# MarvelMathesh/sincformer-metacog-speech-enhancement

Measured on AMD Instinct MI355X. Metric: audio frames/sec/GPU (16 kHz, 512-frame utts) + mask RMSE vs CPU ref, higher is better.
Workload: dtype fp16 MFMA operands (PerceptionAgent, fusion, Conformer GEMMs, heads) + bf16 attention core, fp32 accumulate (ops.POLICIES['mixed']); 1 GPU; B256 x 512-frame utterances (L40880, T512) forward; batch_per_gpu=256, samples=40880, frames_per_utt=512, launch=eager launches, streams=3, precision_policy=mixed

## Files before the change

### sincformer_metacog_speech_enhancement_amd/csrc/headpool.hip

```cpp
#include "sfm_common.h"

#define HP_BM 128
#define HP_K 256
#define HP_STAGE 32768
#define HP_NSTAGE 3
#define HP_IMG 16384


template <class T>
__global__ __launch_bounds__(512) void headpool_kernel(const u16* __restrict__ A, const u16* __restrict__ W,
                                                       const float* __restrict__ bias, u16* __restrict__ pooled,
                                                       float* __restrict__ gn_partial, int Tin, int Tout, int NW, int lda,
                                                       int ldp, int fpt, int P, int gcols, int w_bytes, int p_bytes) {
  extern __shared__ __attribute__((aligned(16))) unsigned char smem[];
  unsigned char* img0 = smem + HP_NSTAGE * HP_STAGE;
  float* bs = reinterpret_cast<float*>(img0 + 2 * HP_IMG);
  float* st = bs + NW;

  const int tid = threadIdx.x, lane = tid & 63;
  const int wave = __builtin_amdgcn_readfirstlane(tid >> 6);
  const int l31 = lane & 31, hl = lane >> 5;
  const int j = blockIdx.x % P, b = blockIdx.x / P;
  const int i0 = j * fpt, i1 = min(i0 + fpt, Tout);
  const int r_lo = (int)(((long long)i0 * Tin) / Tout);
  const int own_end = (j + 1 < P) ? (int)(((long long)i1 * Tin) / Tout) : Tin;
  const int nch = NW >> 6;
  const int ngr = NW / gcols;
  auto a_rs = __builtin_amdgcn_make_buffer_rsrc((void*)(A + (long long)b * Tin * lda), 0, Tin * lda * 2, 0x00020000);
  auto w_rs = __builtin_amdgcn_make_buffer_rsrc((void*)W, 0, w_bytes, 0x00020000);
  auto p_rs = __builtin_amdgcn_make_buffer_rsrc((void*)pooled, 0, p_bytes, 0x00020000);

#pragma unroll
  for (int i = 0; i < 8; ++i) {
    const int inst = wave * 8 + i;
    const int row = inst * 2 + (lane >> 5);
    const int lc = (lane & 31) ^ (row & 15);
    const int r = r_lo + row;
    __builtin_amdgcn_raw_ptr_buffer_load_lds(a_rs, (lds_ptr_t)(smem + inst * 1024), 16,
                                             r < Tin ? (r * lda + lc * 8) * 2 : Tin * lda * 2, 0, 0, 0);
  }
  for (int i = tid; i < NW; i += 512) bs[i] = bias ? bias[i] : 0.f;
  wait_vmcnt<0>();
  __syncthreads();
  const int r1 = (wave >> 1) * 32 + l31;
  u32x4 hf[16];
#pragma unroll
  for (int s = 0; s < 16; ++s) hf[s] = *reinterpret_cast<const u32x4*>(smem + r1 * 512 + (((2 * s + hl) ^ (r1 & 15)) << 4));
  __syncthreads();

  auto w_piece = [&](int c, int stage, int i) {
    const int inst = wave * 4 + i;
    const int row = inst * 2 + (lane >> 5);
    const int lc = (lane & 31) ^ (row & 15);
    const int voff = c < nch ? ((c * 64 + row) * HP_K + lc * 8) * 2 : w_bytes;
    __builtin_amdgcn_raw_ptr_buffer_load_lds(w_rs, (lds_ptr_t)(smem + stage * HP_STAGE + inst * 1024), 16, voff, 0, 0, 0);
  };
#pragma unroll
  for (int c = 0; c < 3; ++c)
#pragma unroll
    for (int i = 0; i < 4; ++i) w_piece(c, c, i);

  const int half = wave & 1;
  const int n1 = half * 32 + l31;
  const uint32_t w_lane = (uint32_t)(uintptr_t)(lds_ptr_t)smem + (uint32_t)(n1 * 512);
  const int hx4 = (hl ^ (n1 & 15)) << 4;
  const bool own = (r_lo + r1) < own_end;
  float gs[2] = {0.f, 0.f}, gq[2] = {0.f, 0.f};
  auto epi_quad = [&](const f32x16& s, int c, int q) {
    const f32x4 bv = *reinterpret_cast<const f32x4*>(bs + c * 64 + half * 32 + 8 * q + 4 * hl);
    float y[4];
#pragma unroll
    for (int e = 0; e < 4; ++e) y[e] = s[4 * q + e] + bv[e];
    u32x2 pk;
    pk[0] = pack2<T>(y[0], y[1]);
    pk[1] = pack2<T>(y[2], y[3]);
    const int col = half * 32 + 8 * q + 4 * hl;
    unsigned char* img = img0 + ((c & 1) ? HP_IMG : 0);
    *reinterpret_cast<u32x2*>(img + r1 * 128 + (((col >> 3) ^ ((r1 >> 1) & 7)) << 4) + (col & 7) * 2) = pk;
    if (own) {
      const int g = (8 * q) / gcols;
#pragma unroll
      for (int e = 0; e < 4; ++e) {
        gs[g] += y[e];
        gq[g] = __builtin_fmaf(y[e], y[e], gq[g]);
      }
    }
  };
  auto stats_out = [&](int c) {
#pragma unroll
    for (int g = 0; g < 2; ++g) {
      const float a = wave_sum_dpp(gs[g]), q2 = wave_sum_dpp(gq[g]);
      if (lane == 0) {
        float* d = st + (((wave >> 1) * ngr + (c * 64 + half * 32) / gcols + g) << 1);
        d[0] = a;
        d[1] = q2;
      }
      gs[g] = 0.f;
      gq[g] = 0.f;
    }
  };
  const int pf = tid >> 4, pc = tid & 15;
  const int fi = i0 + pf;
  int ws = 0, we = 0;
  if (fi < i1) {
    ws = (int)(((long long)fi * Tin) / Tout) - r_lo;
    we = (int)((((long long)(fi + 1)) * Tin + Tout - 1) / Tout) - r_lo;
  }
  const float winv = we > ws ? 1.0f / (float)(we - ws) : 0.f;
  auto pool_chunk = [&](int c) {
    const unsigned char* img = img0 + ((c & 1) ? HP_IMG : 0);
    float a[4] = {0.f, 0.f, 0.f, 0.f};
    for (int r = ws; r < we; ++r) {
      const u32x2 v = *reinterpret_cast<const u32x2*>(img + r * 128 + (((pc >> 1) ^ ((r >> 1) & 7)) << 4) + (pc & 1) * 8);
#pragma unroll
      for (int e = 0; e < 2; ++e) {
        const uint32_t w = v[e];
        a[2 * e] += T::to_f32((u16)(w & 0xffffu));
        a[2 * e + 1] += T::to_f32((u16)(w >> 16));
      }
    }
    u32x2 pk;
    pk[0] = pack2<T>(a[0] * winv, a[1] * winv);
    pk[1] = pack2<T>(a[2] * winv, a[3] * winv);
    const int voff = (fi < i1) ? (((b * Tout + fi) * ldp) + c * 64 + pc * 4) * 2 : p_bytes;
    __builtin_amdgcn_raw_buffer_store_b64(pk, p_rs, voff, 0, 0);
  };

  wait_vmcnt<8>();
  ring_barrier();
  f32x16 s1;
#pragma unroll
  for (int r = 0; r < 16; ++r) s1[r] = 0.f;
  {
    u32x4 fw[4];
#pragma unroll
    for (int k = 0; k < 4; ++k) fw[k] = *reinterpret_cast<const u32x4*>(smem + n1 * 512 + (((2 * k + hl) ^ (n1 & 15)) << 4));
#pragma unroll
    for (int k = 0; k < 16; ++k) {
      s1 = T::mfma(fw[k & 3], hf[k], s1);
      if (k + 4 < 16) fw[k & 3] = *reinterpret_cast<const u32x4*>(smem + n1 * 512 + (((2 * (k + 4) + hl) ^ (n1 & 15)) << 4));
    }
  }
  wait_vmcnt<4>();
  ring_barrier();

  int stage_next = 1, stage_free = 0;
  for (int c = 0; c + 1 < nch; ++c) {
    if (c >= 1) pool_chunk(c - 1);
    f32x16 s1n;
#pragma unroll
    for (int r = 0; r < 16; ++r) s1n[r] = 0.f;
    const uint32_t fbase = w_lane + (uint32_t)(stage_next * HP_STAGE);
    u32x4 fw[4];
#pragma unroll
    for (int k = 0; k < 4; ++k) frag_read(fw[k], fbase + (uint32_t)(hx4 ^ (k << 5)));
#pragma unroll
    for (int k = 0; k < 16; ++k) {
      if (k <= 12) frag_wait<3>(fw[k & 3]);
      else if (k == 13) frag_wait<2>(fw[k & 3]);
      else if (k == 14) frag_wait<1>(fw[k & 3]);
      else frag_wait<0>(fw[k & 3]);
      s1n = T::mfma(fw[k & 3], hf[k], s1n);
      if (k + 4 < 16) frag_read(fw[k & 3], fbase + (uint32_t)(hx4 ^ ((k + 4) << 5)));
      if ((k & 3) == 1) epi_quad(s1, c, k >> 2);
      if ((k & 3) == 3) w_piece(c + 3, stage_free, k >> 2);
    }
    stats_out(c);
    s1 = s1n;
    if (c >= 1) wait_vmcnt<5>();
    else wait_vmcnt<4>();
    ring_barrier();
    stage_free = stage_next;
    stage_next = (stage_next == HP_NSTAGE - 1) ? 0 : stage_next + 1;
  }
  if (nch >= 2) pool_chunk(nch - 2);
#pragma unroll
  for (int q = 0; q < 4; ++q) epi_quad(s1, nch - 1, q);
  stats_out(nch - 1);
  wait_vmcnt<0>();
  ring_barrier();
  pool_chunk(nch - 1);
  if (tid < ngr * 2) {
    const float v = ((st[tid] + st[ngr * 2 + tid]) + st[2 * ngr * 2 + tid]) + st[3 * ngr * 2 + tid];
    gn_partial[((long long)b * P + j) * ngr * 2 + tid] = v;
  }
}

extern "C" int sfm_headpool_frames_per_tile(int Tin, int Tout) {
  if (Tin <= 0 || Tout <= 0 || Tin < Tout) return 0;
  for (int f = 32; f >= 1; --f) {
    bool ok = true;
    for (int i0 = 0; i0 < Tout && ok; i0 += f) {
      const int i1 = i0 + f < Tout ? i0 + f : Tout;
      const long long lo = ((long long)i0 * Tin) / Tout, hi = (((long long)i1) * Tin + Tout - 1) / Tout;
      if (hi - lo > HP_BM) ok = false;
    }
    if (ok) return f;
  }
  return 0;
}

extern "C" int sfm_headpool(const void* xd, const void* W, const float* bias, void* pooled, float* gn_partial, int B, int Tin,
                            int Tout, int NW, int lda, int ldp, int gcols, int dtype, void* stream) {
  if (!xd || !W || !pooled || !gn_partial) return SFM_ERR_ARG;
  if (dtype != SFM_DT_BF16 && dtype != SFM_DT_F16) return SFM_ERR_ARG;
  const int fpt = sfm_headpool_frames_per_tile(Tin, Tout);
  if (B <= 0 || fpt <= 0 || NW <= 0 || (NW % 64) != 0 || NW > 1024 || gcols != 16 || lda < HP_K || (lda % 8) != 0 || (ldp % 4) != 0 ||
      ldp < NW)
    return SFM_ERR_SHAPE;
  const int P = (Tout + fpt - 1) / fpt;
  const long long p_bytes = (long long)B * Tout * ldp * 2, a_b = (long long)Tin * lda * 2;
  if (p_bytes >= (1LL << 31) || a_b >= (1LL << 31) || (long long)B * P > 2147483647LL) return SFM_ERR_SHAPE;
  const int ngr = NW / gcols;
  const int lds = HP_NSTAGE * HP_STAGE + 2 * HP_IMG + NW * 4 + 4 * ngr * 2 * 4;
  const int w_bytes = NW * HP_K * 2;
  dim3 grid(B * P), block(512);
  hipStream_t st = (hipStream_t)stream;
#define HP_GO(TT) SFM_LAUNCH_LDS((headpool_kernel<TT>), grid, block, lds, st, (const u16*)xd, (const u16*)W, bias, (u16*)pooled, gn_partial, \
                                 Tin, Tout, NW, lda, ldp, fpt, P, gcols, w_bytes, (int)p_bytes)
  if (dtype == SFM_DT_F16) HP_GO(F16);
  else HP_GO(BF16);
#undef HP_GO
  return SFM_OK;
}
```

### sincformer_metacog_speech_enhancement_amd/csrc/lin256.hip

```cpp
#include "sfm_common.h"
#include "gemm16_epi.h"

#define L2_BM 128
#define L2_K 256
#define L2_STAGE 32768
#define L2_NSTAGE 3
#define L2_IMG 16384


struct L2Ln {
  const float* x;
  const float* w;
  const float* b;
  int ldx;
  float eps;
};
template <class T, int GLU, int OTHER, int LN>
__global__ __launch_bounds__(512) void lin256_kernel(const u16* __restrict__ A, const u16* __restrict__ W,
                                                     const float* __restrict__ bias, u16* __restrict__ out, int M, int NW,
                                                     int lda, int ldo, int a_bytes, int w_bytes, int o_bytes, L2Ln ln) {
  extern __shared__ __attribute__((aligned(16))) unsigned char smem[];
  unsigned char* img0 = smem + L2_NSTAGE * L2_STAGE;
  float* bs = reinterpret_cast<float*>(img0 + 2 * L2_IMG);
  constexpr int CPG = GLU ? 2 : 1;

  const int tid = threadIdx.x, lane = tid & 63;
  const int wave = __builtin_amdgcn_readfirstlane(tid >> 6);
  const int l31 = lane & 31, hl = lane >> 5;
  const int m0 = blockIdx.x * L2_BM;
  const int nch = NW >> 6;
  auto a_rs = __builtin_amdgcn_make_buffer_rsrc((void*)A, 0, a_bytes, 0x00020000);
  auto w_rs = __builtin_amdgcn_make_buffer_rsrc((void*)W, 0, w_bytes, 0x00020000);
  auto o_rs = __builtin_amdgcn_make_buffer_rsrc((void*)out, 0, o_bytes, 0x00020000);

  if constexpr (LN) {
    const f32x4 gw = *reinterpret_cast<const f32x4*>(ln.w + 4 * lane), gb = *reinterpret_cast<const f32x4*>(ln.b + 4 * lane);
    f32x4 xv[16];
#pragma unroll
    for (int r = 0; r < 16; ++r) {
      int m = m0 + wave * 16 + r;
      m = m < M ? m : M - 1;
      xv[r] = *reinterpret_cast<const f32x4*>(ln.x + (long long)m * ln.ldx + 4 * lane);
    }
#pragma unroll
    for (int r = 0; r < 16; ++r) {
      const int row = wave * 16 + r;
      const f32x4 v = xv[r];
      const float mean = wave_sum_dpp((v[0] + v[1]) + (v[2] + v[3])) * (1.0f / 256.0f);
      float d[4];
#pragma unroll
      for (int j = 0; j < 4; ++j) d[j] = v[j] - mean;
      const float rstd = rsqrtf(wave_sum_dpp((d[0] * d[0] + d[1] * d[1]) + (d[2] * d[2] + d[3] * d[3])) * (1.0f / 256.0f) + ln.eps);
      float y[4];
#pragma unroll
      for (int j = 0; j < 4; ++j) y[j] = d[j] * rstd * gw[j] + gb[j];
      u32x2 pk;
      pk[0] = pack2<T>(y[0], y[1]);
      pk[1] = pack2<T>(y[2], y[3]);
      *reinterpret_cast<u32x2*>(smem + row * 512 + (((lane >> 1) ^ (row & 15)) << 4) + (lane & 1) * 8) = pk;
    }
  } else {
#pragma unroll
    for (int i = 0; i < 8; ++i) {
      const int inst = wave * 8 + i;
      const int row = inst * 2 + (lane >> 5);
      const int lc = (lane & 31) ^ (row & 15);
      const long long voff = ((long long)(m0 + row) * lda + lc * 8) * 2;
      __builtin_amdgcn_raw_ptr_buffer_load_lds(a_rs, (lds_ptr_t)(smem + inst * 1024), 16,
                                               voff < a_bytes ? (int)voff : a_bytes, 0, 0, 0);
    }
  }
  for (int i = tid; i < NW; i += 512) bs[i] = bias ? bias[i] : 0.f;
  wait_vmcnt<0>();
  __syncthreads();
  const int r1 = (wave >> 1) * 32 + l31;
  u32x4 hf[16];
#pragma unroll
  for (int s = 0; s < 16; ++s) hf[s] = *reinterpret_cast<const u32x4*>(smem + r1 * 512 + (((2 * s + hl) ^ (r1 & 15)) << 4));
  __syncthreads();

  auto w_piece = [&](int c, int stage, int i) {
    const int inst = wave * 4 + i;
    const int row = inst * 2 + (lane >> 5);
    const int lc = (lane & 31) ^ (row & 15);
    const int voff = c < nch ? ((c * 64 + row) * L2_K + lc * 8) * 2 : w_bytes;
    __builtin_amdgcn_raw_ptr_buffer_load_lds(w_rs, (lds_ptr_t)(smem + stage * L2_STAGE + inst * 1024), 16, voff, 0, 0, 0);
  };
#pragma unroll
  for (int c = 0; c < 3; ++c)
#pragma unroll
    for (int i = 0; i < 4; ++i) w_piece(c, c, i);

  const int half = wave & 1;
  const int n1 = GLU ? (half * 16 + l31 + ((l31 >= 16) ? 16 : 0)) : (half * 32 + l31);
  const uint32_t w_lane = (uint32_t)(uintptr_t)(lds_ptr_t)smem + (uint32_t)(n1 * 512);
  const int hx4 = (hl ^ (n1 & 15)) << 4;
  auto unit_row = [&](int q) { return GLU ? (half * 16 + 8 * (q & 1) + 4 * hl + ((q >= 2) ? 32 : 0)) : (half * 32 + 8 * q + 4 * hl); };
  auto s_init = [&](int, f32x16& s) {
#pragma unroll
    for (int r = 0; r < 16; ++r) s[r] = 0.f;
  };
  constexpr bool other = OTHER == 1;
  static_assert(!(GLU && OTHER == 2), "fp32 result: plain epilogue only");
  auto epi_quad = [&](const f32x16& s, int c, int q) {
    float y[4];
    int col;
    const f32x4 bv = *reinterpret_cast<const f32x4*>(bs + c * 64 + unit_row(q));
    if (GLU) {
      if (q >= 2) return;
      const f32x4 bg = *reinterpret_cast<const f32x4*>(bs + c * 64 + unit_row(q + 2));
#pragma unroll
      for (int e = 0; e < 4; ++e) y[e] = (s[4 * q + e] + bv[e]) * __builtin_amdgcn_rcpf(1.0f + __expf(-(s[4 * (q + 2) + e] + bg[e])));
      col = (c & 1) * 32 + half * 16 + 8 * q + 4 * hl;
    } else {
#pragma unroll
      for (int e = 0; e < 4; ++e) y[e] = s[4 * q + e] + bv[e];
      col = half * 32 + 8 * q + 4 * hl;
    }
    if constexpr (OTHER == 2) {
      unsigned char* img = img0 + (half ? L2_IMG : 0);
      const int ch = 2 * q + hl;
      *reinterpret_cast<f32x4*>(img + r1 * 128 + ((ch ^ ((r1 >> 1) & 7)) << 4)) = f32x4{y[0], y[1], y[2], y[3]};
      return;
    }
    u32x2 pk;
    pk[0] = pack2_out<T>(y[0], y[1], other);
    pk[1] = pack2_out<T>(y[2], y[3], other);
    unsigned char* img = img0 + (((c / CPG) & 1) ? L2_IMG : 0);
    *reinterpret_cast<u32x2*>(img + r1 * 128 + (((col >> 3) ^ ((r1 >> 1) & 7)) << 4) + (col & 7) * 2) = pk;
  };
  const int ocols = GLU ? (NW >> 1) : NW;
  auto store_group = [&](int g) {
    const unsigned char* img = img0 + ((g & 1) ? L2_IMG : 0);
#pragma unroll
    for (int i = 0; i < 2; ++i) {
      const int idx = tid + 512 * i;
      const int row = idx >> 3, pc = idx & 7;
      const int lc = pc ^ ((row >> 1) & 7);
      const u32x4 v = *reinterpret_cast<const u32x4*>(img + row * 128 + pc * 16);
      const int m = m0 + row, n = g * 64 + lc * 8;
      const int voff = (m < M && n < ocols) ? (m * ldo + n) * 2 : o_bytes;
      __builtin_amdgcn_raw_buffer_store_b128(v, o_rs, voff, 0, 0);
    }
  };

  auto store_chunk32 = [&](int c) {
#pragma unroll
    for (int i = 0; i < 2; ++i)
#pragma unroll
      for (int j = 0; j < 2; ++j) {
        const int idx = tid + 512 * j;
        const int row = idx >> 3, pc = idx & 7;
        const int lc = pc ^ ((row >> 1) & 7);
        const u32x4 v = *reinterpret_cast<const u32x4*>(img0 + (i ? L2_IMG : 0) + row * 128 + pc * 16);
        const int m = m0 + row, n = c * 64 + i * 32 + lc * 4;
        const int voff = (m < M && n < ocols) ? (m * ldo + n) * 4 : o_bytes;
        __builtin_amdgcn_raw_buffer_store_b128(v, o_rs, voff, 0, 0);
      }
  };

  wait_vmcnt<8>();
  ring_barrier();
  f32x16 s1;
  s_init(0, s1);
  {
    u32x4 fw[4];
#pragma unroll
    for (int k = 0; k < 4; ++k) fw[k] = *reinterpret_cast<const u32x4*>(smem + n1 * 512 + (((2 * k + hl) ^ (n1 & 15)) << 4));
#pragma unroll
    for (int k = 0; k < 16; ++k) {
      s1 = T::mfma(fw[k & 3], hf[k], s1);
      if (k + 4 < 16) fw[k & 3] = *reinterpret_cast<const u32x4*>(smem + n1 * 512 + (((2 * (k + 4) + hl) ^ (n1 & 15)) << 4));
    }
  }
  wait_vmcnt<4>();
  ring_barrier();

  int stage_next = 1;
  int stage_free = 0;
  int stored = 0;
  for (int c = 0; c + 1 < nch; ++c) {
    bool did_store = false;
    if constexpr (OTHER == 2) {
      if (c >= 1) {
        store_chunk32(c - 1);
        ring_barrier();
      }
    }
    if (OTHER != 2 && c >= CPG && (c % CPG) == 0) {
      store_group(stored);
      ++stored;
      did_store = true;
    }
    f32x16 s1n;
    s_init(c + 1, s1n);
    const uint32_t fbase = w_lane + (uint32_t)(stage_next * L2_STAGE);
    u32x4 fw[4];
#pragma unroll
    for (int k = 0; k < 4; ++k) frag_read(fw[k], fbase + (uint32_t)(hx4 ^ (k << 5)));
#pragma unroll
    for (int k = 0; k < 16; ++k) {
      if (k <= 12) frag_wait<3>(fw[k & 3]);
      else if (k == 13) frag_wait<2>(fw[k & 3]);
      else if (k == 14) frag_wait<1>(fw[k & 3]);
      else frag_wait<0>(fw[k & 3]);
      s1n = T::mfma(fw[k & 3], hf[k], s1n);
      if (k + 4 < 16) frag_read(fw[k & 3], fbase + (uint32_t)(hx4 ^ ((k + 4) << 5)));
      if ((k & 3) == 1) epi_quad(s1, c, k >> 2);
      if ((k & 3) == 3) w_piece(c + 3, stage_free, k >> 2);
    }
    s1 = s1n;
    if (OTHER == 2) wait_vmcnt<8>();
    else if (did_store) wait_vmcnt<6>();
    else wait_vmcnt<4>();
    ring_barrier();
    stage_free = stage_next;
    stage_next = (stage_next == L2_NSTAGE - 1) ? 0 : stage_next + 1;
  }
  if constexpr (OTHER == 2) {
    if (nch >= 2) {
      store_chunk32(nch - 2);
      ring_barrier();
    }
  }
#pragma unroll
  for (int q = 0; q < 4; ++q) epi_quad(s1, nch - 1, q);
  wait_vmcnt<0>();
  ring_barrier();
  if constexpr (OTHER == 2) {
    store_chunk32(nch - 1);
  } else {
    const int ngroups = (nch + CPG - 1) / CPG;
    for (; stored < ngroups; ++stored) store_group(stored);
  }
}

static int lin256_launch(const void* A, const float* X32, int ldx, const float* lnw, const float* lnb, float eps, const void* W,
                         const float* bias, void* out, int M, int NW, int lda, int ldo, int glu, int dtype, int out_dtype,
                         void* stream) {
  const bool has_ln = X32 != nullptr;
  if ((!A && !has_ln) || !W || !out || (has_ln && (!lnw || !lnb))) return SFM_ERR_ARG;
  if ((dtype != SFM_DT_BF16 && dtype != SFM_DT_F16) || (out_dtype != SFM_DT_BF16 && out_dtype != SFM_DT_F16 && out_dtype != 2))
    return SFM_ERR_ARG;
  const bool f32o = out_dtype == 2;
  if (M <= 0 || NW <= 0 || (NW % 64) != 0 || NW > 2048 || (glu && ((NW % 128) != 0 || f32o)) || (ldo % (f32o ? 4 : 8)) != 0 ||
      ldo < (glu ? NW / 2 : NW))
    return SFM_ERR_SHAPE;
  if (has_ln ? (ldx < L2_K || (ldx % 4) != 0 || f32o || (((uintptr_t)X32 | (uintptr_t)lnw | (uintptr_t)lnb) % 16) != 0)
             : (lda < L2_K || (lda % 8) != 0))
    return SFM_ERR_SHAPE;
  const long long a_bytes = has_ln ? 0 : (long long)(M - 1) * lda * 2 + L2_K * 2;
  const long long o_bytes = ((long long)(M - 1) * ldo + (glu ? NW / 2 : NW)) * (f32o ? 4 : 2);
  if (a_bytes >= (1LL << 31) || o_bytes >= (1LL << 31)) return SFM_ERR_SHAPE;
  const int lds = L2_NSTAGE * L2_STAGE + 2 * L2_IMG + NW * 4;
  const int w_bytes = NW * L2_K * 2;
  const int other = f32o ? 2 : (out_dtype != dtype ? 1 : 0);
  dim3 grid((M + L2_BM - 1) / L2_BM), block(512);
  hipStream_t st = (hipStream_t)stream;
  const int ki = (has_ln ? 12 : 0) + (dtype == SFM_DT_F16 ? 6 : 0) + (glu ? 3 : 0) + other;
  const L2Ln ln = {X32, lnw, lnb, ldx, eps};
#define L2_GO(TT, G, O, N) SFM_LAUNCH_LDS((lin256_kernel<TT, G, O, N>), grid, block, lds, st, (const u16*)A, (const u16*)W, bias, (u16*)out, \
                                          M, NW, lda, ldo, (int)a_bytes, w_bytes, (int)o_bytes, ln)
  switch (ki) {
    case 0: L2_GO(BF16, 0, 0, 0); break;
    case 1: L2_GO(BF16, 0, 1, 0); break;
    case 2: L2_GO(BF16, 0, 2, 0); break;
    case 3: L2_GO(BF16, 1, 0, 0); break;
    case 4: L2_GO(BF16, 1, 1, 0); break;
    case 6: L2_GO(F16, 0, 0, 0); break;
    case 7: L2_GO(F16, 0, 1, 0); break;
    case 8: L2_GO(F16, 0, 2, 0); break;
    case 9: L2_GO(F16, 1, 0, 0); break;
    case 10: L2_GO(F16, 1, 1, 0); break;
    case 12: L2_GO(BF16, 0, 0, 1); break;
    case 13: L2_GO(BF16, 0, 1, 1); break;
    case 15: L2_GO(BF16, 1, 0, 1); break;
    case 16: L2_GO(BF16, 1, 1, 1); break;
    case 18: L2_GO(F16, 0, 0, 1); break;
    case 19: L2_GO(F16, 0, 1, 1); break;
    case 21: L2_GO(F16, 1, 0, 1); break;
    case 22: L2_GO(F16, 1, 1, 1); break;
    default: return SFM_ERR_SHAPE;
  }
#undef L2_GO
  return SFM_OK;
}

extern "C" int sfm_lin256(const void* A, const void* W, const float* bias, void* out, int M, int NW, int lda, int ldo, int glu,
                          int dtype, int out_dtype, void* stream) {
  return lin256_launch(A, nullptr, 0, nullptr, nullptr, 0.f, W, bias, out, M, NW, lda, ldo, glu, dtype, out_dtype, stream);
}

extern "C" int sfm_ln_lin256(const float* X32, int ldx, const float* lnw, const float* lnb, float eps, const void* W,
                             const float* bias, void* out, int M, int NW, int ldo, int glu, int dtype, int out_dtype, void* stream) {
  if (!X32) return SFM_ERR_ARG;
  return lin256_launch(nullptr, X32, ldx, lnw, lnb, eps, W, bias, out, M, NW, 0, ldo, glu, dtype, out_dtype, stream);
}
```

Before: 9.373 million STFT frames/s (whole job).

## Halve block size and weight chunk width in headpool/lin256; per-wave output strips

Both kernels drop from 512 to 256 threads, each wave now owns 32 rows of the 128-row tile, and weight chunks shrink from 64 to 32 columns, halving the LDS stage and image buffers. The aim is to fit two blocks per CU and cut LDS footprint. In lin256 the shared double-buffered output image becomes a per-wave 4 KB strip, flushed by each wave on its own, which removes block-wide barriers around stores. This costs twice as many chunk iterations, plus extra ring barriers and MFMA rounds per output column, and the GLU weight-row remapping risks indexing mistakes.

Result: no change. 9.344 million STFT frames/s (whole job) (-0.3%).

```diff
diff --git a/sincformer_metacog_speech_enhancement_amd/csrc/headpool.hip b/sincformer_metacog_speech_enhancement_amd/csrc/headpool.hip
--- a/sincformer_metacog_speech_enhancement_amd/csrc/headpool.hip
+++ b/sincformer_metacog_speech_enhancement_amd/csrc/headpool.hip
@@ -2,16 +2,19 @@
 
 #define HP_BM 128
 #define HP_K 256
-#define HP_STAGE 32768
+#define HP_CH 32
+#define HP_STAGE 16384
 #define HP_NSTAGE 3
-#define HP_IMG 16384
+#define HP_IMG 8192
+#define HP_THREADS 256
 
 
 template <class T>
-__global__ __launch_bounds__(512) void headpool_kernel(const u16* __restrict__ A, const u16* __restrict__ W,
-                                                       const float* __restrict__ bias, u16* __restrict__ pooled,
-                                                       float* __restrict__ gn_partial, int Tin, int Tout, int NW, int lda,
-                                                       int ldp, int fpt, int P, int gcols, int w_bytes, int p_bytes) {
+__global__ __launch_bounds__(HP_THREADS, 2) void headpool_kernel(const u16* __restrict__ A, const u16* __restrict__ W,
+                                                                 const float* __restrict__ bias, u16* __restrict__ pooled,
+                                                                 float* __restrict__ gn_partial, int Tin, int Tout, int NW,
+                                                                 int lda, int ldp, int fpt, int P, int gcols, int w_bytes,
+                                                                 int p_bytes) {
   extern __shared__ __attribute__((aligned(16))) unsigned char smem[];
   unsigned char* img0 = smem + HP_NSTAGE * HP_STAGE;
   float* bs = reinterpret_cast<float*>(img0 + 2 * HP_IMG);
@@ -24,25 +27,25 @@
   const int i0 = j * fpt, i1 = min(i0 + fpt, Tout);
   const int r_lo = (int)(((long long)i0 * Tin) / Tout);
   const int own_end = (j + 1 < P) ? (int)(((long long)i1 * Tin) / Tout) : Tin;
-  const int nch = NW >> 6;
+  const int nch = NW >> 5;
   const int ngr = NW / gcols;
   auto a_rs = __builtin_amdgcn_make_buffer_rsrc((void*)(A + (long long)b * Tin * lda), 0, Tin * lda * 2, 0x00020000);
   auto w_rs = __builtin_amdgcn_make_buffer_rsrc((void*)W, 0, w_bytes, 0x00020000);
   auto p_rs = __builtin_amdgcn_make_buffer_rsrc((void*)pooled, 0, p_bytes, 0x00020000);
 
 #pragma unroll
-  for (int i = 0; i < 8; ++i) {
-    const int inst = wave * 8 + i;
+  for (int i = 0; i < 16; ++i) {
+    const int inst = wave * 16 + i;
     const int row = inst * 2 + (lane >> 5);
     const int lc = (lane & 31) ^ (row & 15);
     const int r = r_lo + row;
     __builtin_amdgcn_raw_ptr_buffer_load_lds(a_rs, (lds_ptr_t)(smem + inst * 1024), 16,
                                              r < Tin ? (r * lda + lc * 8) * 2 : Tin * lda * 2, 0, 0, 0);
   }
-  for (int i = tid; i < NW; i += 512) bs[i] = bias ? bias[i] : 0.f;
+  for (int i = tid; i < NW; i += HP_THREADS) bs[i] = bias ? bias[i] : 0.f;
   wait_vmcnt<0>();
   __syncthreads();
-  const int r1 = (wave >> 1) * 32 + l31;
+  const int r1 = wave * 32 + l31;
   u32x4 hf[16];
 #pragma unroll
   for (int s = 0; s < 16; ++s) hf[s] = *reinterpret_cast<const u32x4*>(smem + r1 * 512 + (((2 * s + hl) ^ (r1 & 15)) << 4));
@@ -52,7 +55,7 @@
     const int inst = wave * 4 + i;
     const int row = inst * 2 + (lane >> 5);
     const int lc = (lane & 31) ^ (row & 15);
-    const int voff = c < nch ? ((c * 64 + row) * HP_K + lc * 8) * 2 : w_bytes;
+    const int voff = c < nch ? ((c * HP_CH + row) * HP_K + lc * 8) * 2 : w_bytes;
     __builtin_amdgcn_raw_ptr_buffer_load_lds(w_rs, (lds_ptr_t)(smem + stage * HP_STAGE + inst * 1024), 16, voff, 0, 0, 0);
   };
 #pragma unroll
@@ -60,23 +63,21 @@
 #pragma unroll
     for (int i = 0; i < 4; ++i) w_piece(c, c, i);
 
-  const int half = wave & 1;
-  const int n1 = half * 32 + l31;
+  const int n1 = l31;
   const uint32_t w_lane = (uint32_t)(uintptr_t)(lds_ptr_t)smem + (uint32_t)(n1 * 512);
   const int hx4 = (hl ^ (n1 & 15)) << 4;
   const bool own = (r_lo + r1) < own_end;
   float gs[2] = {0.f, 0.f}, gq[2] = {0.f, 0.f};
   auto epi_quad = [&](const f32x16& s, int c, int q) {
-    const f32x4 bv = *reinterpret_cast<const f32x4*>(bs + c * 64 + half * 32 + 8 * q + 4 * hl);
+    const f32x4 bv = *reinterpret_cast<const f32x4*>(bs + c * HP_CH + 8 * q + 4 * hl);
     float y[4];
 #pragma unroll
     for (int e = 0; e < 4; ++e) y[e] = s[4 * q + e] + bv[e];
     u32x2 pk;
     pk[0] = pack2<T>(y[0], y[1]);
     pk[1] = pack2<T>(y[2], y[3]);
-    const int col = half * 32 + 8 * q + 4 * hl;
     unsigned char* img = img0 + ((c & 1) ? HP_IMG : 0);
-    *reinterpret_cast<u32x2*>(img + r1 * 128 + (((col >> 3) ^ ((r1 >> 1) & 7)) << 4) + (col & 7) * 2) = pk;
+    *reinterpret_cast<u32x2*>(img + r1 * 64 + ((q ^ ((r1 >> 2) & 3)) << 4) + hl * 8) = pk;
     if (own) {
       const int g = (8 * q) / gcols;
 #pragma unroll
@@ -91,7 +92,7 @@
     for (int g = 0; g < 2; ++g) {
       const float a = wave_sum_dpp(gs[g]), q2 = wave_sum_dpp(gq[g]);
       if (lane == 0) {
-        float* d = st + (((wave >> 1) * ngr + (c * 64 + half * 32) / gcols + g) << 1);
+        float* d = st + ((wave * ngr + (c * HP_CH) / gcols + g) << 1);
         d[0] = a;
         d[1] = q2;
       }
@@ -99,7 +100,7 @@
       gq[g] = 0.f;
     }
   };
-  const int pf = tid >> 4, pc = tid & 15;
+  const int pf = tid >> 3, pc = tid & 7;
   const int fi = i0 + pf;
   int ws = 0, we = 0;
   if (fi < i1) {
@@ -111,7 +112,7 @@
     const unsigned char* img = img0 + ((c & 1) ? HP_IMG : 0);
     float a[4] = {0.f, 0.f, 0.f, 0.f};
     for (int r = ws; r < we; ++r) {
-      const u32x2 v = *reinterpret_cast<const u32x2*>(img + r * 128 + (((pc >> 1) ^ ((r >> 1) & 7)) << 4) + (pc & 1) * 8);
+      const u32x2 v = *reinterpret_cast<const u32x2*>(img + r * 64 + (((pc >> 1) ^ ((r >> 2) & 3)) << 4) + (pc & 1) * 8);
 #pragma unroll
       for (int e = 0; e < 2; ++e) {
         const uint32_t w = v[e];
@@ -122,7 +123,7 @@
     u32x2 pk;
     pk[0] = pack2<T>(a[0] * winv, a[1] * winv);
     pk[1] = pack2<T>(a[2] * winv, a[3] * winv);
-    const int voff = (fi < i1) ? (((b * Tout + fi) * ldp) + c * 64 + pc * 4) * 2 : p_bytes;
+    const int voff = (fi < i1) ? (((b * Tout + fi) * ldp) + c * HP_CH + pc * 4) * 2 : p_bytes;
     __builtin_amdgcn_raw_buffer_store_b64(pk, p_rs, voff, 0, 0);
   };
 
@@ -214,7 +215,7 @@
   const int ngr = NW / gcols;
   const int lds = HP_NSTAGE * HP_STAGE + 2 * HP_IMG + NW * 4 + 4 * ngr * 2 * 4;
   const int w_bytes = NW * HP_K * 2;
-  dim3 grid(B * P), block(512);
+  dim3 grid(B * P), block(HP_THREADS);
   hipStream_t st = (hipStream_t)stream;
 #define HP_GO(TT) SFM_LAUNCH_LDS((headpool_kernel<TT>), grid, block, lds, st, (const u16*)xd, (const u16*)W, bias, (u16*)pooled, gn_partial, \
                                  Tin, Tout, NW, lda, ldp, fpt, P, gcols, w_bytes, (int)p_bytes)
diff --git a/sincformer_metacog_speech_enhancement_amd/csrc/lin256.hip b/sincformer_metacog_speech_enhancement_amd/csrc/lin256.hip
--- a/sincformer_metacog_speech_enhancement_amd/csrc/lin256.hip
+++ b/sincformer_metacog_speech_enhancement_amd/csrc/lin256.hip
@@ -3,9 +3,11 @@
 
 #define L2_BM 128
 #define L2_K 256
-#define L2_STAGE 32768
+#define L2_CH 32
+#define L2_STAGE 16384
 #define L2_NSTAGE 3
-#define L2_IMG 16384
+#define L2_STRIP 4096
+#define L2_THREADS 256
 
 
 struct L2Ln {
@@ -16,53 +18,57 @@
   float eps;
 };
 template <class T, int GLU, int OTHER, int LN>
-__global__ __launch_bounds__(512) void lin256_kernel(const u16* __restrict__ A, const u16* __restrict__ W,
-                                                     const float* __restrict__ bias, u16* __restrict__ out, int M, int NW,
-                                                     int lda, int ldo, int a_bytes, int w_bytes, int o_bytes, L2Ln ln) {
+__global__ __launch_bounds__(L2_THREADS, 2) void lin256_kernel(const u16* __restrict__ A, const u16* __restrict__ W,
+                                                               const float* __restrict__ bias, u16* __restrict__ out, int M, int NW,
+                                                               int lda, int ldo, int a_bytes, int w_bytes, int o_bytes, L2Ln ln) {
   extern __shared__ __attribute__((aligned(16))) unsigned char smem[];
-  unsigned char* img0 = smem + L2_NSTAGE * L2_STAGE;
-  float* bs = reinterpret_cast<float*>(img0 + 2 * L2_IMG);
-  constexpr int CPG = GLU ? 2 : 1;
-
   const int tid = threadIdx.x, lane = tid & 63;
   const int wave = __builtin_amdgcn_readfirstlane(tid >> 6);
+  unsigned char* strip = smem + L2_NSTAGE * L2_STAGE + wave * L2_STRIP;
+  float* bs = reinterpret_cast<float*>(smem + L2_NSTAGE * L2_STAGE + 4 * L2_STRIP);
+  static_assert(!(GLU && OTHER == 2), "fp32 result: plain epilogue only");
+  constexpr int CPG = OTHER == 2 ? 1 : (GLU ? 4 : 2);
+
   const int l31 = lane & 31, hl = lane >> 5;
   const int m0 = blockIdx.x * L2_BM;
-  const int nch = NW >> 6;
+  const int nch = NW >> 5;
   auto a_rs = __builtin_amdgcn_make_buffer_rsrc((void*)A, 0, a_bytes, 0x00020000);
   auto w_rs = __builtin_amdgcn_make_buffer_rsrc((void*)W, 0, w_bytes, 0x00020000);
   auto o_rs = __builtin_amdgcn_make_buffer_rsrc((void*)out, 0, o_bytes, 0x00020000);
 
   if constexpr (LN) {
     const f32x4 gw = *reinterpret_cast<const f32x4*>(ln.w + 4 * lane), gb = *reinterpret_cast<const f32x4*>(ln.b + 4 * lane);
-    f32x4 xv[16];
-#pragma unroll
-    for (int r = 0; r < 16; ++r) {
-      int m = m0 + wave * 16 + r;
-      m = m < M ? m : M - 1;
-      xv[r] = *reinterpret_cast<const f32x4*>(ln.x + (long long)m * ln.ldx + 4 * lane);
-    }
-#pragma unroll
-    for (int r = 0; r < 16; ++r) {
-      const int row = wave * 16 + r;
-      const f32x4 v = xv[r];
-      const float mean = wave_sum_dpp((v[0] + v[1]) + (v[2] + v[3])) * (1.0f / 256.0f);
-      float d[4];
-#pragma unroll
-      for (int j = 0; j < 4; ++j) d[j] = v[j] - mean;
-      const float rstd = rsqrtf(wave_sum_dpp((d[0] * d[0] + d[1] * d[1]) + (d[2] * d[2] + d[3] * d[3])) * (1.0f / 256.0f) + ln.eps);
-      float y[4];
-#pragma unroll
-      for (int j = 0; j < 4; ++j) y[j] = d[j] * rstd * gw[j] + gb[j];
-      u32x2 pk;
-      pk[0] = pack2<T>(y[0], y[1]);
-      pk[1] = pack2<T>(y[2], y[3]);
-      *reinterpret_cast<u32x2*>(smem + row * 512 + (((lane >> 1) ^ (row & 15)) << 4) + (lane & 1) * 8) = pk;
+#pragma unroll 1
+    for (int h = 0; h < 2; ++h) {
+      f32x4 xv[16];
+#pragma unroll
+      for (int r = 0; r < 16; ++r) {
+        int m = m0 + wave * 32 + h * 16 + r;
+        m = m < M ? m : M - 1;
+        xv[r] = *reinterpret_cast<const f32x4*>(ln.x + (long long)m * ln.ldx + 4 * lane);
+      }
+#pragma unroll
+      for (int r = 0; r < 16; ++r) {
+        const int row = wave * 32 + h * 16 + r;
+        const f32x4 v = xv[r];
+        const float mean = wave_sum_dpp((v[0] + v[1]) + (v[2] + v[3])) * (1.0f / 256.0f);
+        float d[4];
+#pragma unroll
+        for (int j = 0; j < 4; ++j) d[j] = v[j] - mean;
+        const float rstd = rsqrtf(wave_sum_dpp((d[0] * d[0] + d[1] * d[1]) + (d[2] * d[2] + d[3] * d[3])) * (1.0f / 256.0f) + ln.eps);
+        float y[4];
+#pragma unroll
+        for (int j = 0; j < 4; ++j) y[j] = d[j] * rstd * gw[j] + gb[j];
+        u32x2 pk;
+        pk[0] = pack2<T>(y[0], y[1]);
+        pk[1] = pack2<T>(y[2], y[3]);
+        *reinterpret_cast<u32x2*>(smem + row * 512 + (((lane >> 1) ^ (row & 15)) << 4) + (lane & 1) * 8) = pk;
+      }
     }
   } else {
 #pragma unroll
-    for (int i = 0; i < 8; ++i) {
-      const int inst = wave * 8 + i;
+    for (int i = 0; i < 16; ++i) {
+      const int inst = wave * 16 + i;
       const int row = inst * 2 + (lane >> 5);
       const int lc = (lane & 31) ^ (row & 15);
       const long long voff = ((long long)(m0 + row) * lda + lc * 8) * 2;
@@ -70,10 +76,10 @@
                                                voff < a_bytes ? (int)voff : a_bytes, 0, 0, 0);
     }
   }
-  for (int i = tid; i < NW; i += 512) bs[i] = bias ? bias[i] : 0.f;
+  for (int i = tid; i < NW; i += L2_THREADS) bs[i] = bias ? bias[i] : 0.f;
   wait_vmcnt<0>();
   __syncthreads();
-  const int r1 = (wave >> 1) * 32 + l31;
+  const int r1 = wave * 32 + l31;
   u32x4 hf[16];
 #pragma unroll
   for (int s = 0; s < 16; ++s) hf[s] = *reinterpret_cast<const u32x4*>(smem + r1 * 512 + (((2 * s + hl) ^ (r1 & 15)) << 4));
@@ -83,7 +89,8 @@
     const int inst = wave * 4 + i;
     const int row = inst * 2 + (lane >> 5);
     const int lc = (lane & 31) ^ (row & 15);
-    const int voff = c < nch ? ((c * 64 + row) * L2_K + lc * 8) * 2 : w_bytes;
+    const int wrow = GLU ? ((c >> 1) * 64 + (c & 1) * 16 + (row & 15) + ((row >= 16) ? 32 : 0)) : (c * L2_CH + row);
+    const int voff = c < nch ? (wrow * L2_K + lc * 8) * 2 : w_bytes;
     __builtin_amdgcn_raw_ptr_buffer_load_lds(w_rs, (lds_ptr_t)(smem + stage * L2_STAGE + inst * 1024), 16, voff, 0, 0, 0);
   };
 #pragma unroll
@@ -91,72 +98,59 @@
 #pragma unroll
     for (int i = 0; i < 4; ++i) w_piece(c, c, i);
 
-  const int half = wave & 1;
-  const int n1 = GLU ? (half * 16 + l31 + ((l31 >= 16) ? 16 : 0)) : (half * 32 + l31);
+  const int n1 = l31;
   const uint32_t w_lane = (uint32_t)(uintptr_t)(lds_ptr_t)smem + (uint32_t)(n1 * 512);
   const int hx4 = (hl ^ (n1 & 15)) << 4;
-  auto unit_row = [&](int q) { return GLU ? (half * 16 + 8 * (q & 1) + 4 * hl + ((q >= 2) ? 32 : 0)) : (half * 32 + 8 * q + 4 * hl); };
+  auto unit_row = [&](int c, int q) {
+    return GLU ? ((c >> 1) * 64 + (c & 1) * 16 + 8 * (q & 1) + 4 * hl + ((q >= 2) ? 32 : 0)) : (c * L2_CH + 8 * q + 4 * hl);
+  };
   auto s_init = [&](int, f32x16& s) {
 #pragma unroll
     for (int r = 0; r < 16; ++r) s[r] = 0.f;
   };
   constexpr bool other = OTHER == 1;
-  static_assert(!(GLU && OTHER == 2), "fp32 result: plain epilogue only");
   auto epi_quad = [&](const f32x16& s, int c, int q) {
     float y[4];
     int col;
-    const f32x4 bv = *reinterpret_cast<const f32x4*>(bs + c * 64 + unit_row(q));
+    const f32x4 bv = *reinterpret_cast<const f32x4*>(bs + unit_row(c, q));
     if (GLU) {
       if (q >= 2) return;
-      const f32x4 bg = *reinterpret_cast<const f32x4*>(bs + c * 64 + unit_row(q + 2));
+      const f32x4 bg = *reinterpret_cast<const f32x4*>(bs + unit_row(c, q + 2));
 #pragma unroll
       for (int e = 0; e < 4; ++e) y[e] = (s[4 * q + e] + bv[e]) * __builtin_amdgcn_rcpf(1.0f + __expf(-(s[4 * (q + 2) + e] + bg[e])));
-      col = (c & 1) * 32 + half * 16 + 8 * q + 4 * hl;
+      col = (c & 3) * 16 + 8 * q + 4 * hl;
     } else {
 #pragma unroll
       for (int e = 0; e < 4; ++e) y[e] = s[4 * q + e] + bv[e];
-      col = half * 32 + 8 * q + 4 * hl;
+      col = (c & 1) * 32 + 8 * q + 4 * hl;
     }
     if constexpr (OTHER == 2) {
-      unsigned char* img = img0 + (half ? L2_IMG : 0);
       const int ch = 2 * q + hl;
-      *reinterpret_cast<f32x4*>(img + r1 * 128 + ((ch ^ ((r1 >> 1) & 7)) << 4)) = f32x4{y[0], y[1], y[2], y[3]};
+      *reinterpret_cast<f32x4*>(strip + l31 * 128 + ((ch ^ ((l31 >> 1) & 7)) << 4)) = f32x4{y[0], y[1], y[2], y[3]};
       return;
     }
     u32x2 pk;
     pk[0] = pack2_out<T>(y[0], y[1], other);
     pk[1] = pack2_out<T>(y[2], y[3], other);
-    unsigned char* img = img0 + (((c / CPG) & 1) ? L2_IMG : 0);
-    *reinterpret_cast<u32x2*>(img + r1 * 128 + (((col >> 3) ^ ((r1 >> 1) & 7)) << 4) + (col & 7) * 2) = pk;
+    *reinterpret_cast<u32x2*>(strip + l31 * 128 + (((col >> 3) ^ ((l31 >> 1) & 7)) << 4) + (col & 7) * 2) = pk;
   };
   const int ocols = GLU ? (NW >> 1) : NW;
-  auto store_group = [&](int g) {
-    const unsigned char* img = img0 + ((g & 1) ? L2_IMG : 0);
-#pragma unroll
-    for (int i = 0; i < 2; ++i) {
-      const int idx = tid + 512 * i;
+  constexpr int OSZ = OTHER == 2 ? 4 : 2;
+  constexpr int GCOLS = 128 / OSZ;
+  auto strip_read = [&](u32x4 (&v)[4]) {
+#pragma unroll
+    for (int i = 0; i < 4; ++i) v[i] = *reinterpret_cast<const u32x4*>(strip + (lane + 64 * i) * 16);
+  };
+  auto strip_store = [&](const u32x4 (&v)[4], int g) {
+#pragma unroll
+    for (int i = 0; i < 4; ++i) {
+      const int idx = lane + 64 * i;
       const int row = idx >> 3, pc = idx & 7;
       const int lc = pc ^ ((row >> 1) & 7);
-      const u32x4 v = *reinterpret_cast<const u32x4*>(img + row * 128 + pc * 16);
-      const int m = m0 + row, n = g * 64 + lc * 8;
-      const int voff = (m < M && n < ocols) ? (m * ldo + n) * 2 : o_bytes;
-      __builtin_amdgcn_raw_buffer_store_b128(v, o_rs, voff, 0, 0);
-    }
-  };
-
-  auto store_chunk32 = [&](int c) {
-#pragma unroll
-    for (int i = 0; i < 2; ++i)
-#pragma unroll
-      for (int j = 0; j < 2; ++j) {
-        const int idx = tid + 512 * j;
-        const int row = idx >> 3, pc = idx & 7;
-        const int lc = pc ^ ((row >> 1) & 7);
-        const u32x4 v = *reinterpret_cast<const u32x4*>(img0 + (i ? L2_IMG : 0) + row * 128 + pc * 16);
-        const int m = m0 + row, n = c * 64 + i * 32 + lc * 4;
-        const int voff = (m < M && n < ocols) ? (m * ldo + n) * 4 : o_bytes;
-        __builtin_amdgcn_raw_buffer_store_b128(v, o_rs, voff, 0, 0);
-      }
+      const int m = m0 + wave * 32 + row, n = g * GCOLS + lc * (16 / OSZ);
+      const int voff = (m < M && n < ocols) ? (m * ldo + n) * OSZ : o_bytes;
+      __builtin_amdgcn_raw_buffer_store_b128(v[i], o_rs, voff, 0, 0);
+    }
   };
 
   wait_vmcnt<8>();
@@ -180,24 +174,19 @@
   int stage_free = 0;
   int stored = 0;
   for (int c = 0; c + 1 < nch; ++c) {
-    bool did_store = false;
-    if constexpr (OTHER == 2) {
-      if (c >= 1) {
-        store_chunk32(c - 1);
-        ring_barrier();
-      }
-    }
-    if (OTHER != 2 && c >= CPG && (c % CPG) == 0) {
-      store_group(stored);
-      ++stored;
-      did_store = true;
-    }
+    const bool do_store = c >= CPG && (c % CPG) == 0;
+    u32x4 sv[4];
+    if (do_store) strip_read(sv);
     f32x16 s1n;
     s_init(c + 1, s1n);
     const uint32_t fbase = w_lane + (uint32_t)(stage_next * L2_STAGE);
     u32x4 fw[4];
 #pragma unroll
     for (int k = 0; k < 4; ++k) frag_read(fw[k], fbase + (uint32_t)(hx4 ^ (k << 5)));
+    if (do_store) {
+      strip_store(sv, stored);
+      ++stored;
+    }
 #pragma unroll
     for (int k = 0; k < 16; ++k) {
       if (k <= 12) frag_wait<3>(fw[k & 3]);
@@ -210,28 +199,25 @@
       if ((k & 3) == 3) w_piece(c + 3, stage_free, k >> 2);
     }
     s1 = s1n;
-    if (OTHER == 2) wait_vmcnt<8>();
-    else if (did_store) wait_vmcnt<6>();
+    if (do_store) wait_vmcnt<8>();
     else wait_vmcnt<4>();
     ring_barrier();
     stage_free = stage_next;
     stage_next = (stage_next == L2_NSTAGE - 1) ? 0 : stage_next + 1;
   }
-  if constexpr (OTHER == 2) {
-    if (nch >= 2) {
-      store_chunk32(nch - 2);
-      ring_barrier();
-    }
+  if (nch - 1 >= CPG && ((nch - 1) % CPG) == 0) {
+    u32x4 sv[4];
+    strip_read(sv);
+    strip_store(sv, stored);
+    ++stored;
   }
 #pragma unroll
   for (int q = 0; q < 4; ++q) epi_quad(s1, nch - 1, q);
   wait_vmcnt<0>();
-  ring_barrier();
-  if constexpr (OTHER == 2) {
-    store_chunk32(nch - 1);
-  } else {
-    const int ngroups = (nch + CPG - 1) / CPG;
-    for (; stored < ngroups; ++stored) store_group(stored);
+  {
+    u32x4 sv[4];
+    strip_read(sv);
+    strip_store(sv, stored);
   }
 }
 
@@ -252,10 +238,10 @@
   const long long a_bytes = has_ln ? 0 : (long long)(M - 1) * lda * 2 + L2_K * 2;
   const long long o_bytes = ((long long)(M - 1) * ldo + (glu ? NW / 2 : NW)) * (f32o ? 4 : 2);
   if (a_bytes >= (1LL << 31) || o_bytes >= (1LL << 31)) return SFM_ERR_SHAPE;
-  const int lds = L2_NSTAGE * L2_STAGE + 2 * L2_IMG + NW * 4;
+  const int lds = L2_NSTAGE * L2_STAGE + 4 * L2_STRIP + NW * 4;
   const int w_bytes = NW * L2_K * 2;
   const int other = f32o ? 2 : (out_dtype != dtype ? 1 : 0);
-  dim3 grid((M + L2_BM - 1) / L2_BM), block(512);
+  dim3 grid((M + L2_BM - 1) / L2_BM), block(L2_THREADS);
   hipStream_t st = (hipStream_t)stream;
   const int ki = (has_ln ? 12 : 0) + (dtype == SFM_DT_F16 ? 6 : 0) + (glu ? 3 : 0) + other;
   const L2Ln ln = {X32, lnw, lnb, ldx, eps};
```
